# amathislab/BUCTD

Hardware: AMD Instinct MI355X
Metric: images/sec (train) BUCTD-CoAM-W48 384x288 (higher is better)
Workload: dtype f32 (3x3 convs: operands split exactly into 3 bf16 pieces, 6 bf16 MFMAs per product, fp32 accumulate - fp32-class); 1 GPU; BUCTD-CoAM-W48 (pose_hrnet_coam, ATT_MODULES [F,T,F,F], colored condition) 384x288 CrowdPose-14kpt full train step: fwd + JointsMSE + bwd + grad all-reduce + Adam + arg-max accuracy decode; global_batch=32, batch_per_gpu=32, input=N x 6 x 384 x 288 fp32, params=115581770, parallelism=dp1, hip_streams=4, conv_math=bf16x6, step_graph=False

## Files before the change

### buctd_amd/_C.py

```python
import ctypes as C
import os

import torch

_HERE = os.path.dirname(os.path.abspath(__file__))
LIB_PATH = os.path.join(_HERE, "lib", "libbuctd_hip.so")


class ConvDesc(C.Structure):
    _fields_ = [(n, C.c_int) for n in ("N", "H", "W", "Ci", "Co", "R", "S", "stride", "pad", "Ho", "Wo")]


class BasicBlockDesc(C.Structure):
    _fields_ = ([(n, C.c_int) for n in ("N", "H", "W", "C")] +
                [(n, C.c_void_p) for n in ("x", "w1_fwd", "w2_fwd", "w1_bwd", "w2_bwd", "gamma1", "beta1", "gamma2", "beta2",
                                           "running_mean1", "running_var1", "running_mean2", "running_var2")] +
                [(n, C.c_float) for n in ("eps1", "momentum1", "eps2", "momentum2")] +
                [(n, C.c_void_p) for n in ("z1", "z2", "y", "acc", "stat")])


class BasicBlockGrads(C.Structure):
    _fields_ = ([(n, C.c_void_p) for n in ("dy", "dz2", "dres", "dy1", "dz1", "dx", "dw1", "dw2", "dgamma1", "dbeta1",
                                           "dgamma2", "dbeta2")] +
                [(n, C.c_int) for n in ("acc_w1", "acc_w2", "acc_bn1", "acc_bn2")] +
                [("bn_acc", C.c_void_p), ("wg_ws", C.c_void_p), ("wg_ws_bytes", C.c_size_t)])


class BnAccIn(C.Structure):
    _fields_ = [("acc", C.c_void_p), ("rows", C.c_long), ("eps", C.c_float), ("momentum", C.c_float),
                ("mean_out", C.c_void_p), ("invstd_out", C.c_void_p), ("running_mean", C.c_void_p),
                ("running_var", C.c_void_p)]


class C3Conv(C.Structure):
    _fields_ = ([(n, C.c_int) for n in ("N", "H", "W", "Ci", "Co")] +
                [(n, C.c_void_p) for n in ("x", "wprep", "residual")] + [("relu", C.c_int)] +
                [(n, C.c_void_p) for n in ("y", "stats_acc")] + [("in_bn", C.POINTER(BnAccIn))] +
                [(n, C.c_void_p) for n in ("in_gamma", "in_beta")] + [("in_relu", C.c_int)] +
                [(n, C.c_void_p) for n in ("bn_z", "bn_y", "bn_mean", "bn_invstd", "bn_gamma", "bn_beta", "bn_acc")])


class C3ConvEval(C.Structure):
    _fields_ = ([(n, C.c_int) for n in ("N", "H", "W", "Ci", "Co")] +
                [(n, C.c_void_p) for n in ("x", "wprep", "scale", "shift", "residual")] + [("relu", C.c_int), ("y", C.c_void_p)])


class BnApplyItem(C.Structure):
    _fields_ = [("z", C.c_void_p), ("st", BnAccIn), ("gamma", C.c_void_p), ("beta", C.c_void_p), ("residual", C.c_void_p),
                ("relu", C.c_int), ("y", C.c_void_p), ("rows", C.c_long), ("C", C.c_int)]


class BnBwdItem(C.Structure):
    _fields_ = ([(n, C.c_void_p) for n in ("dy", "y", "z", "mean", "invstd", "gamma", "beta")] +
                [("relu", C.c_int), ("rows", C.c_long), ("C", C.c_int)] +
                [(n, C.c_void_p) for n in ("dz", "dres", "dgamma", "dbeta")] +
                [("accumulate", C.c_int), ("acc", C.c_void_p), ("acc_ready", C.c_int)])


class Wg3Conv(C.Structure):
    _fields_ = ([(n, C.c_int) for n in ("N", "H", "W", "Ci", "Co")] +
                [(n, C.c_void_p) for n in ("x", "dy", "dw")] + [("accumulate", C.c_int)] +
                [(n, C.c_void_p) for n in ("x_mean", "x_invstd", "x_gamma", "x_beta")] + [("x_relu", C.c_int)] +
                [("workspace", C.c_void_p), ("workspace_bytes", C.c_size_t)])


class MhaArgs(C.Structure):
    _fields_ = ([(n, C.c_int) for n in ("B", "T", "h", "dh")] +
                [(n, C.c_void_p) for n in ("q", "k", "v")] + [(n, C.c_int) for n in ("ldq", "ldk", "ldv")] +
                [("out", C.c_void_p), ("ldo", C.c_int), ("lse", C.c_void_p), ("scale", C.c_float), ("p_drop", C.c_float),
                 ("dout", C.c_void_p), ("lddo", C.c_int)] +
                [(n, C.c_void_p) for n in ("dq", "dk", "dv")] + [(n, C.c_int) for n in ("lddq", "lddk", "lddv")])


class AttnRowsArgs(C.Structure):
    _fields_ = ([(n, C.c_int) for n in ("B", "T", "h", "dh", "R")] + [("q", C.c_void_p), ("k", C.c_void_p)] +
                [("ldq", C.c_int), ("ldk", C.c_int), ("rows", C.c_void_p), ("scale", C.c_float), ("out", C.c_void_p),
                 ("out_heads", C.c_void_p)])


class RefineArgs(C.Structure):
    _fields_ = ([(n, C.c_void_p) for n in ("coords", "maxvals", "offset", "center", "scale", "box_score", "items",
                                           "cond_trunc", "cond_joints", "status", "hist_preds", "hist_score",
                                           "hist_box_score", "hist_keypoint_score", "hist_center", "hist_scale")] +
                [(n, C.c_int) for n in ("B", "K", "pass_", "passes", "heatmap_w", "heatmap_h", "crop_w", "crop_h")] +
                [(n, C.c_double) for n in ("margin", "aspect_ratio", "in_vis_thre", "scale_thre")])


class SampleGeomArgs(C.Structure):
    _fields_ = ([(n, C.c_void_p) for n in ("joints", "joints_vis", "cond", "cond_vis", "center", "scale", "bbox",
                                           "half_body", "draws", "bbox_draws", "flags", "pair", "items", "out_joints",
                                           "out_joints_vis", "out_cond", "out_cond_vis", "cond_trunc", "target_xy",
                                           "target_vis", "out_center", "out_scale", "out_rotation", "status")] +
                [(n, C.c_int) for n in ("B", "K", "crop_w", "crop_h", "keep_rect", "bbox_aug")] +
                [(n, C.c_double) for n in ("margin", "aspect_ratio", "scale_thre", "stride_x", "stride_y")])


class KptMatchArgs(C.Structure):
    _fields_ = ([(n, C.c_int) for n in ("images", "K", "n_thr", "n_area")] + [(n, C.c_long) for n in ("dt_total", "gt_total")] +
                [(n, C.c_void_p) for n in ("dt_offsets", "gt_offsets", "oks_offsets", "dt_kpts", "gt_kpts", "gt_area",
                                           "gt_bbox", "gt_flags", "sigmas", "thresholds", "area_ranges", "oks",
                                           "dt_matched", "dt_ignored")])


class VisCanvas(C.Structure):
    _fields_ = [("base", C.c_void_p), ("row_stride", C.c_long), ("H", C.c_int), ("W", C.c_int)]


class VisPoseArgs(C.Structure):
    _fields_ = ([(n, C.c_void_p) for n in ("canvases", "person_offsets", "persons", "joints", "skeleton", "palette",
                                           "tiles")] +
                [(n, C.c_int) for n in ("C", "P", "K", "L", "n_palette", "n_tiles", "canvas_h_max", "canvas_w_max",
                                        "style", "thickness", "radius")] +
                [("score_thresh", C.c_float), ("alpha256", C.c_int)])


VIS_POSE_PLAIN, VIS_POSE_PRETTY = 0, 1
# ... 62 lines not shown
    "buctd_bn_finalize": (_I, [_P, _P, _I, _I, _L, _I, _F, _F, _P, _P, _P, _P, _P]),
    "buctd_conv3x3_bf16x3_supported": (_I, [_I, _I, _I, _I, _I]),
    "buctd_conv3x3_bf16x3_stats_groups": (_I, [_I, _I, _I, _I, _I, _PI, _PI]),
    "buctd_conv3x3_bf16x3_prep_bytes": (_SZ, [_I, _I, _I]),
    "buctd_conv3x3_bf16x3_prep": (_I, [_I, _I, _P, _I, _P, _P]),
    "buctd_conv3x3_bf16x3_prep_batched": (_I, [_P, _I, _L, _P]),
    "buctd_conv3x3_bf16x3": (_I, [_I, _I, _I, _I, _I, _P, _P, _P, _P, _P, _P, _I, _P, _P, _P, _P]),
    "buctd_conv3x3_wgrad_bf16x3_supported": (_I, [_I, _I, _I, _I, _I]),
    "buctd_conv3x3_wgrad_bf16x3_workspace": (_SZ, [_I, _I, _I, _I, _I]),
    "buctd_conv3x3_wgrad_bf16x3": (_I, [_I, _I, _I, _I, _I, _P, _P, _P, _I, _P, _SZ, _P]),
    "buctd_conv3x3_bf16x6_supported": (_I, [_I, _I, _I, _I, _I]),
    "buctd_conv3x3_bf16x6_stats_groups": (_I, [_I, _I, _I, _I, _I, _PI, _PI]),
    "buctd_conv3x3_bf16x6_prep_bytes": (_SZ, [_I, _I, _I]),
    "buctd_conv3x3_bf16x6_prep": (_I, [_I, _I, _P, _I, _P, _P]),
    "buctd_conv3x3_bf16x6": (_I, [_I, _I, _I, _I, _I, _P, _P, _P, _P, _P, _P, _I, _P, _P, _P, _P]),
    "buctd_bn_bwd_from_partials": (_I, [_P, _P, _P, _P, _P, _P, _P, _I, _L, _I, _P, _I, _P, _P, _P, _P, _I, _P, _SZ, _P]),
    "buctd_conv3x3_wgrad_bf16x6_bnin": (_I, [_I, _I, _I, _I, _I, _P, _P, _P, _I, _P, _P, _P, _P, _I, _P, _SZ, _P]),
    "buctd_conv3x3_wgrad_bf16x6_supported": (_I, [_I, _I, _I, _I, _I]),
    "buctd_conv3x3_wgrad_bf16x6_workspace": (_SZ, [_I, _I, _I, _I, _I]),
    "buctd_conv3x3_wgrad_bf16x6": (_I, [_I, _I, _I, _I, _I, _P, _P, _P, _I, _P, _SZ, _P]),
    "buctd_bn_stats": (_I, [_P, _L, _I, _P, _PI, _PI, _P]),
    "buctd_bn_stats_groups": (_I, [_L, _I, _PI, _PI]),
    "buctd_bn_apply": (_I, [_P, _P, _P, _P, _P, _P, _I, _P, _L, _I, _P]),
    "buctd_bn_bwd_workspace": (_SZ, [_L, _I]),
    "buctd_bn_bwd": (_I, [_P, _P, _P, _P, _P, _P, _P, _I, _L, _I, _P, _P, _P, _P, _I, _P, _SZ, _P]),
    "buctd_bn_fold": (_I, [_P, _P, _P, _P, _F, _I, _P, _P, _P]),
    "buctd_bn_acc_bytes": (_SZ, [_I]),
    "buctd_bn_apply_acc": (_I, [_P, C.POINTER(BnAccIn), _P, _P, _P, _I, _P, _L, _I, _P]),
    "buctd_bn_bwd_acc": (_I, [_P, _P, _P, _P, _P, _P, _P, _I, _L, _I, _P, _P, _P, _P, _I, _P, _I, _P]),
    "buctd_conv3x3_bf16x6_acc": (_I, [_I] * 5 + [_P, _P, _P, _I, _P, _P, C.POINTER(BnAccIn), _P, _P, _I, _P]),
    "buctd_conv3x3_bf16x6_bnstat_acc": (_I, [_I] * 5 + [_P] * 12),
    "buctd_gconv_x6_fwd_acc": (_I, [_I] * 6 + [_P] * 6),
    "buctd_conv3x3_bf16x6_group": (_I, [_I, C.POINTER(C3Conv), _P]),
    "buctd_conv3x3_bf16x6_group_eval": (_I, [_I, C.POINTER(C3ConvEval), _P]),
    "buctd_conv3x3_bf16x6_group_workgroups": (_I, [_I, C.POINTER(C3Conv)]),
    "buctd_conv3x3_bf16x6_group_plan": (_I, [_I, C.POINTER(C3Conv), C.POINTER(C.c_int)]),
    "buctd_conv3x3_bf16x6_plan": (_I, [_I, _I, _I, _I, _I, _I, C.POINTER(C.c_int)]),
    "buctd_conv3x3_wgrad_bf16x6_plan": (_I, [_I, _I, _I, _I, _I, C.POINTER(C.c_int)]),
    "buctd_gconv_wgrad_x6_supported": (_I, [_I] * 6),
    "buctd_gconv_wgrad_x6_plan": (_I, [_I] * 6 + [C.POINTER(C.c_int)]),
    "buctd_gconv_wgrad_x6_workspace": (_SZ, [_I] * 6),
    "buctd_gconv_wgrad_x6": (_I, [_I] * 6 + [_P, _P, _P, _I, _P, _SZ, _P]),
    "buctd_bn_apply_acc_group": (_I, [_I, C.POINTER(BnApplyItem), _P]),
    "buctd_bn_bwd_acc_group": (_I, [_I, C.POINTER(BnBwdItem), _P]),
    "buctd_conv3x3_wgrad_bf16x6_group_workspace": (_SZ, [_I] * 6),
    "buctd_conv3x3_wgrad_bf16x6_group": (_I, [_I, C.POINTER(Wg3Conv), _P]),
    "buctd_conv3x3_wgrad_bf16x6_group_workgroups": (_I, [_I, C.POINTER(Wg3Conv)]),
    "buctd_conv3x3_wgrad_bf16x6_group_plan": (_I, [_I, C.POINTER(Wg3Conv), C.POINTER(C.c_int)]),
    "buctd_stream_fork": (_I, [_P, _P]),
    "buctd_basic_branches_fwd_train": (_I, [_I, _I, C.POINTER(BasicBlockDesc), _P]),
    "buctd_basic_branches_bwd": (_I, [_I, _I, C.POINTER(BasicBlockDesc), C.POINTER(BasicBlockGrads), _P, _P]),
    "buctd_basic_chain_fwd_train": (_I, [_I, C.POINTER(BasicBlockDesc), _P]),
    "buctd_basic_chain_bwd": (_I, [_I, C.POINTER(BasicBlockDesc), C.POINTER(BasicBlockGrads), _P, _P]),
    "buctd_x6_image_dims": (_I, [_I, _I, _I, _P, _P]),
    "buctd_x6_image_bytes": (C.c_size_t, [_I, _I, _I]),
    "buctd_x6_image": (_I, [_P, _I, _I, _I, _L, _L, _I, _L, _L, _I, _P, _P]),
    "buctd_x6_gemm": (_I, [_I, _I, _I, _P, _P, _P, _I, _F, _P, _L, _I, _L, _P]),
    "buctd_x6_gemm_plan": (_I, [_I, _I, _I, _PI]),
    "buctd_x6_gemm_tile": (_I, [_I, _I, _I, _I, _PI, _PI]),
    "buctd_x6_image_path": (_I, [_P, _I, _I, _I, _L, _L, _I, _L, _L, _I, _I, _I, _PI]),
    "buctd_add": (_I, [_P, _P, _P, _L, _I, _P]),
    "buctd_add_n": (_I, [C.POINTER(_P), _I, _P, _L, _P]),
    "buctd_mul": (_I, [_P, _P, _P, _L, _P]),
    "buctd_scale": (_I, [_P, _P, _F, _P, _L, _P]),
    "buctd_copy_channels": (_I, [_P, _L, _I, _I, _P, _I, _I, _I, _P]),
    "buctd_add_bcast": (_I, [_P, _P, _P, _L, _L, _P]),
    "buctd_batch_sum": (_I, [_P, _L, _L, _P, _I, _P]),
    "buctd_relu_bwd": (_I, [_P, _P, _P, _L, _P]),
    "buctd_colsum_workspace": (_SZ, [_L, _I]),
    "buctd_colsum": (_I, [_P, _L, _I, _P, _I, _P, _SZ, _P]),
    "buctd_nchw_to_nhwc": (_I, [_P, _I, _I, _I, _I, _I, _I, _P, _P]),
    "buctd_nhwc_to_nchw": (_I, [_P, _I, _I, _I, _I, _P, _P]),
    "buctd_fuse_sum": (_I, [C.POINTER(_P), _PI, _I, _I, _I, _I, _I, _I, _P, _P]),
    "buctd_fuse_sum_bwd": (_I, [_P, _P, _I, _I, _I, _I, _I, _P, _P]),
    "buctd_resize_bilinear": (_I, [_P, _I, _I, _I, _I, _I, _I, _I, _I, _P, _P]),
    "buctd_maxpool3x3s2_fwd": (_I, [_P, _I, _I, _I, _I, _P, _P, _P]),
    "buctd_maxpool3x3s2_bwd": (_I, [_P, _P, _I, _I, _I, _I, _P, _P]),
    "buctd_softmax_dropout_fwd": (_I, [_P, _L, _I, _F, _F, _U64, _P, _P, _P]),
    "buctd_softmax_dropout_bwd": (_I, [_P, _P, _L, _I, _F, _F, _U64, _P, _P]),
    "buctd_softmax_dropout_fwd_dseed": (_I, [_P, _L, _I, _F, _F, _P, _P, _P, _P]),
    "buctd_softmax_dropout_bwd_dseed": (_I, [_P, _P, _L, _I, _F, _F, _P, _P, _P]),
    "buctd_dropout": (_I, [_P, _P, _L, _F, _U64, _P]),
    "buctd_dropout_dseed": (_I, [_P, _P, _L, _F, _P, _P]),
    "buctd_dropout_seed_fill": (_I, [_P, _I, _U64, _U64, _P]),
    "buctd_attn_smallqk_supported": (_I, [_I, _I, _I]),
    "buctd_attn_smallqk_plan": (_I, [_I, _I, _I, _I, _F, _I, _PI]),
    "buctd_attn_smallqk_fwd": (_I, [_I, _I, _I, _I, _P, _P, _P, _F, _F, _U64, _I, _P, _P, _P, _P]),
    "buctd_attn_smallqk_bwd": (_I, [_I, _I, _I, _I, _P, _P, _P, _P, _P, _P, _P, _F, _F, _U64, _I, _P, _P, _P, _P, _P]),
    "buctd_attn_smallqk_fwd_dseed": (_I, [_I, _I, _I, _I, _P, _P, _P, _F, _F, _P, _I, _P, _P, _P, _P]),
    "buctd_attn_smallqk_bwd_dseed": (_I, [_I, _I, _I, _I, _P, _P, _P, _P, _P, _P, _P, _F, _F, _P, _I, _P, _P, _P, _P, _P]),
    "buctd_layernorm_fwd": (_I, [_P, _P, _P, _L, _I, _F, _P, _P, _P, _P]),
    "buctd_add_layernorm_fwd": (_I, [_P, _P, _P, _P, _L, _I, _F, _P, _P, _P, _P, _P]),
    "buctd_layernorm_bwd_workspace": (_SZ, [_L, _I]),
    "buctd_layernorm_bwd": (_I, [_P, _P, _P, _P, _P, _L, _I, _P, _P, _P, _I, _P, _SZ, _P]),
    "buctd_joints_mse": (_I, [_P, _P, _P, _I, _I, _I, _P, _P, _F, _P, _SZ, _P]),
    "buctd_joints_ohkm_mse_workspace": (_SZ, [_I, _I]),
    "buctd_joints_ohkm_mse": (_I, [_P, _P, _P, _I, _I, _I, _I, _P, _P, _F, _P, _SZ, _P]),
    "buctd_argmax_decode": (_I, [_P, _I, _I, _I, _P, _P, _P, _P]),
    "buctd_warp_affine_norm": (_I, [_P, _I, _I, _I, _P, _P, _P, _L, _P, _P]),
    "buctd_cond_render_into": (_I, [_P, _I, _P, _I, _I, _I, _I, _I, _I, _P, _L, _P, _SZ, _P]),
    "buctd_cond_geometry": (_I, [_P, _P, _P, _P, _I, _I, _P, _P, _P, _P]),
    "buctd_cond_mirror": (_I, [_P, _I, _P, _P, _I, _I, _I, _P, _P]),
    "buctd_mirror_rows": (_I, [_P, _L, _P, _L, _P, _I, _I, _I, _I, _I, _P]),
    "buctd_refine_step": (_I, [C.POINTER(RefineArgs), _P]),
    "buctd_sample_geometry": (_I, [C.POINTER(SampleGeomArgs), _P]),
    "buctd_synthesize_pose": (_I, [_P, _P, _P, _P, _P, _P, _I, _I, _I, C.c_ulonglong, _P, _P]),
# ... 117 lines not shown
```

### buctd_amd/models/hrnet_common.py

```python
import logging
import os

import torch

from .. import nn
from .. import ops

BN_MOMENTUM = 0.1
logger = logging.getLogger(__name__)


def conv3x3(in_planes, out_planes, stride=1):
    return nn.Conv2d(in_planes, out_planes, kernel_size=3, stride=stride, padding=1, bias=False)


class BasicBlock(nn.Module):
    expansion = 1

    def __init__(self, inplanes, planes, stride=1, downsample=None):
        super().__init__()
        self.conv1 = conv3x3(inplanes, planes, stride)
        self.bn1 = nn.BatchNorm2d(planes, momentum=BN_MOMENTUM)
        self.relu = nn.ReLU(inplace=True)
        self.conv2 = conv3x3(planes, planes)
# ... 128 lines not shown
            rows.append(nn.ModuleList(row))
        return nn.ModuleList(rows)

    def get_num_inchannels(self):
        return self.num_inchannels

    def _branches_grouped(self, x):
        nb = self.num_branches
        if not (self.training and torch.is_grad_enabled() and all(type(br) is BlockChain and len(br) > 1 for br in self.branches)):
            return None
        chains = []
        for br in self.branches:
            if not all(_native_block(m) and m.bn1.track_running_stats == br[0].bn1.track_running_stats for m in br):
                return None
            chains.append([_block_params(m) for m in br])
        xs = [x[i] for i in range(nb)]
        if not ops.group_branches_ok(xs, chains):
            return None
        parts = ops.group_branch_partition(nb)
        if len(parts) == 1:
            return list(ops.BasicBranchesFn.apply(chains[0][0][0], chains, *xs))
        outs = ops.fork_join([lambda p=p: ops.BasicBranchesFn.apply(chains[p[0]][0][0], [chains[i] for i in p], *[xs[i] for i in p])
                              for p in parts], [[xs[i] for i in p] for p in parts])
        ys = [None] * nb
        for p, o in zip(parts, outs):
            for i, y in zip(p, o):
                ys[i] = y
        return ys

    def _branches_grouped_eval(self, x):
        if self.training or torch.is_grad_enabled() or not all(type(br) is BlockChain and len(br) > 0 for br in self.branches):
            return None
        chains = []
        for br in self.branches:
            if not all(type(m) is BasicBlock and m.downsample is None and m.stride == 1 and m.conv1.bias is None
                       and m.conv2.bias is None and not m.bn1.training and not m.bn2.training
                       and m.bn1.running_mean is not None and m.bn2.running_mean is not None for m in br):
                return None
            chains.append([_block_params(m) for m in br])
        xs = [x[i] for i in range(self.num_branches)]
        if not ops.eval_branches_ok(xs, chains):
            return None
        return ops.basic_branches_eval(xs, chains)

    def forward(self, x):
        if self.num_branches == 1:
            return [self.branches[0](x[0])]
        xs = self._branches_grouped(x)
        if xs is None:
            xs = self._branches_grouped_eval(x)
        if xs is None:
            xs = ops.fork_join([lambda i=i: self.branches[i](x[i]) for i in range(self.num_branches)],
                               [x[i] for i in range(self.num_branches)])
        rows = list(enumerate(self.fuse_layers))
        fan = len(rows) > 1 and torch.is_grad_enabled() and any(t.requires_grad for t in xs)
        xr = [ops.FanOut.apply(xs[j], len(rows)) if fan and xs[j].is_cuda else [xs[j]] * len(rows)
              for j in range(self.num_branches)]

        def fuse_row(i, row):
            terms, shifts = [], []
            for j in range(self.num_branches):
                if j == i:
                    terms.append(xr[j][i])
                    shifts.append(0)
                elif j > i:
                    terms.append(row[j](xr[j][i]))
                    shifts.append(j - i)
                else:
                    terms.append(row[j](xr[j][i]))
                    shifts.append(0)
            return ops.FuseSum.apply(tuple(shifts), True, *terms)

        return ops.fork_join([lambda i=i, row=row: fuse_row(i, row) for i, row in rows], [xs for _ in rows], tag=1)


def make_transition_layer(pre, cur):
    layers = []
    for i in range(len(cur)):
        if i < len(pre):
            if cur[i] != pre[i]:
                layers.append(nn.ConvBN(nn.Conv2d(pre[i], cur[i], 3, 1, 1, bias=False), nn.BatchNorm2d(cur[i]),
                                        nn.ReLU(inplace=True)))
            else:
                layers.append(None)
        else:
            steps = []
            for j in range(i + 1 - len(pre)):
                cin = pre[-1]
                cout = cur[i] if j == i - len(pre) else cin
                steps.append(nn.ConvBN(nn.Conv2d(cin, cout, 3, 2, 1, bias=False), nn.BatchNorm2d(cout),
                                       nn.ReLU(inplace=True)))
            layers.append(nn.Chain(*steps))
    return nn.ModuleList(layers)


def make_stage(layer_config, num_inchannels, multi_scale_output=True):
    block = blocks_dict[layer_config["BLOCK"]]
    modules = []
    for i in range(layer_config["NUM_MODULES"]):
        mso = multi_scale_output or i != layer_config["NUM_MODULES"] - 1
        modules.append(HighResolutionModule(layer_config["NUM_BRANCHES"], block, layer_config["NUM_BLOCKS"],
                                            num_inchannels, layer_config["NUM_CHANNELS"],
                                            layer_config["FUSE_METHOD"], mso))
        num_inchannels = modules[-1].get_num_inchannels()
    return nn.Chain(*modules), num_inchannels


class HRNetTrunk(nn.Module):

    def build_trunk(self, extra, last_stage=4):
        self.conv1 = nn.Conv2d(3, 64, kernel_size=3, stride=2, padding=1, bias=False)
        self.bn1 = nn.BatchNorm2d(64, momentum=BN_MOMENTUM)
# ... 71 lines not shown
```

### buctd_amd/ops.py

```python
import ctypes as C
import math
import weakref

import torch

from . import _C
from ._C import ConvDesc, MatmulDesc, check, lib, ptr, stream_ptr

_capture = {"on": False, "events": set(), "allow_seeds": False, "seed_table": None, "seed_draws": 0}
_SEED_TABLE_SLOTS = 1024


def capturing():
    return _capture["on"]


def _new_event(stream=None):
    ev = torch.cuda.Event()
    ev.record(stream) if stream is not None else ev.record()
    if _capture["on"]:
        _capture["events"].add(id(ev))
        _capture.setdefault("keep", []).append(ev)
    return ev

# ... 1939 lines not shown
        return (None, None) + tuple(tmps[b][0, _Chain.DX] if ctx.needs_input_grad[2 + b] else None for b in range(nb))


class Conv(torch.autograd.Function):

    @staticmethod
    def forward(ctx, x, w, b, stride, pad, relu):
        y = conv_fwd(x, w, b, stride, pad, relu=relu)
        ctx.meta = (w, b, stride, pad, relu, tuple(x.shape))
        ctx.save_for_backward(x, y if relu else None)
        return y

    @staticmethod
    def backward(ctx, dy):
        w, b, stride, pad, relu, x_shape = ctx.meta
        x, y = ctx.saved_tensors
        dy = _contig(dy)
        if relu:
            dy = relu_bwd(dy, y)
        dx = conv_dgrad(dy, w, x_shape, stride, pad) if ctx.needs_input_grad[0] else None
        if w.requires_grad:
            dw, acc = grad_target(w)
            conv_wgrad_async(x, dy, w, stride, pad, dw, acc)
        if b is not None and b.requires_grad:
            db, acc = grad_target(b)
            colsum(dy, dy.shape[-1], db, acc)
        grad_done(w, b)
        return dx, None, None, None, None, None


class FuseSum(torch.autograd.Function):

    @staticmethod
    def forward(ctx, shifts, relu, *terms):
        out = fuse_sum(list(terms), list(shifts), relu)
        ctx.shifts, ctx.relu = shifts, relu
        ctx.save_for_backward(out if relu else None)
        return out

    @staticmethod
    def backward(ctx, dy):
        (y,) = ctx.saved_tensors
        dy = _contig(dy)
        cache = {}
        grads = []
        for j, s in enumerate(ctx.shifts):
            if not ctx.needs_input_grad[2 + j]:
                grads.append(None)
                continue
            if s not in cache:
                cache[s] = fuse_sum_bwd(dy, y, s) if s > 0 or ctx.relu else dy
            grads.append(cache[s])
        return (None, None, *grads)


class AddN(torch.autograd.Function):

    @staticmethod
    def forward(ctx, a, b, c):
        out = add(a, b)
        if c is not None:
            out = add(out, c, out=out)
        ctx.n = 3 if c is not None else 2
        return out

    @staticmethod
    def backward(ctx, dy):
        return dy, dy, (dy if ctx.n == 3 else None)


def add_n(terms):
    acc = terms[0]
    k = 1
    while k < len(terms):
        group = [acc] + list(terms[k:k + 3])
        k += 3
        out = torch.empty_like(acc)
        arr = (C.c_void_p * len(group))(*[t.data_ptr() for t in group])
        check(lib().buctd_add_n(arr, len(group), ptr(out), acc.numel(), stream_ptr()), "add_n")
        acc = out
    return acc


class FanOut(torch.autograd.Function):

    @staticmethod
    def forward(ctx, x, n):
        return tuple(x.view_as(x) for _ in range(n))

    @staticmethod
    def backward(ctx, *grads):
        gs = [_contig(g) for g in grads if g is not None]
        if not gs:
            return None, None
        return (gs[0] if len(gs) == 1 else add_n(gs)), None


class ToNCHW(torch.autograd.Function):
    @staticmethod
    def forward(ctx, x):
        return nhwc_to_nchw(x)

    @staticmethod
    def backward(ctx, dy):
        return nchw_to_nhwc(_contig(dy))

# ... 397 lines not shown
```

### include/buctd_hip.h

```cpp
#ifndef BUCTD_HIP_H
#define BUCTD_HIP_H
#include <stddef.h>
#include <stdint.h>

#ifdef __cplusplus
extern "C" {
#endif

int buctd_version(void);
const char* buctd_last_error(void);

typedef struct {
  int N, H, W, Ci;
  int Co, R, S;
  int stride, pad;
  int Ho, Wo;
} buctd_conv_desc;

int buctd_conv2d_fwd_thin(const buctd_conv_desc* d);
int buctd_conv2d_fwd(const buctd_conv_desc* d, const float* x, const float* w, const float* bias,
                     const float* scale, const float* shift, const float* residual, int relu, float* y,
                     float* stats_partials, void* stream);
int buctd_conv2d_dgrad(const buctd_conv_desc* d, const float* dy, const float* w, const float* bias, float* dx,
                       float* stats_partials, void* stream);
// ... 248 lines not shown
int buctd_flipback_avg(const float* a, const float* b, const int32_t* perm, int N, int K, int H, int W, int shift,
                       float* out, void* stream);

int buctd_gconv_x6_supported(int kind, int N, int H, int W, int Ci, int Co, int dir);
size_t buctd_gconv_x6_prep_bytes(int kind, int Ci, int Co, int dir);
int buctd_gconv_x6_prep(int kind, int Ci, int Co, const float* w, int dir, void* wprep, void* stream);
size_t buctd_gconv_x6_prep_item_bytes(void);
int buctd_gconv_x6_prep_item(int kind, int Ci, int Co, const float* w, int dir, void* wprep, void* item_host);
int buctd_gconv_x6_prep_batched(const void* items_device, int n, void* stream);
int buctd_gconv_x6_stats_groups(int kind, int N, int H, int W, int Ci, int Co, int* ngroups, int* rows_per_group);
int buctd_gconv_x6_fwd(int kind, int N, int H, int W, int Ci, int Co, const float* x, const void* wprep, const float* bias,
                       const float* scale, const float* shift, const float* residual, int relu, float* y,
                       float* stats_partials, int* stats_counts, void* stream);
int buctd_gconv_x6_fwd_acc(int kind, int N, int H, int W, int Ci, int Co, const float* x, const void* wprep, const float* bias,
                           float* y, void* stats_acc, void* stream);
int buctd_gconv_x6_dgrad(int kind, int N, int H, int W, int Ci, int Co, const float* dy, const void* wprep,
                         const float* residual, float* dx, void* stream);
int buctd_gconv_x6_plan(int kind, int dir, int N, int H, int W, int Ci, int Co, int flags, int* out);
int buctd_gconv_wgrad_x6_supported(int kind, int N, int H, int W, int Ci, int Co);
int buctd_gconv_wgrad_x6_plan(int kind, int N, int H, int W, int Ci, int Co, int* out);
size_t buctd_gconv_wgrad_x6_workspace(int kind, int N, int H, int W, int Ci, int Co);
int buctd_gconv_wgrad_x6(int kind, int N, int H, int W, int Ci, int Co, const float* x, const float* dy, float* dw,
                         int accumulate, void* workspace, size_t workspace_bytes, void* stream);

typedef struct {
  int N, H, W, C;
  const float* x;
  const void *w1_fwd, *w2_fwd;
  const void *w1_bwd, *w2_bwd;
  const float *gamma1, *beta1, *gamma2, *beta2;
  float *running_mean1, *running_var1, *running_mean2, *running_var2;
  float eps1, momentum1, eps2, momentum2;
  float *z1, *z2, *y;
  void* acc;
  float* stat;
} buctd_basic_block;
typedef struct {
  const float* dy;
  float *dz2, *dres, *dy1, *dz1;
  float* dx;
  float *dw1, *dw2, *dgamma1, *dbeta1, *dgamma2, *dbeta2;
  int acc_w1, acc_w2, acc_bn1, acc_bn2;
  void* bn_acc;
  void* wg_ws; size_t wg_ws_bytes;
} buctd_basic_block_grads;
int buctd_basic_chain_fwd_train(int n, const buctd_basic_block* blocks, void* stream);
int buctd_basic_chain_bwd(int n, const buctd_basic_block* blocks, const buctd_basic_block_grads* grads, void* stream,
                          void* side_stream);

int buctd_basic_branches_fwd_train(int nb, int n, const buctd_basic_block* blocks, void* stream);
int buctd_basic_branches_bwd(int nb, int n, const buctd_basic_block* blocks, const buctd_basic_block_grads* grads, void* stream,
                             void* side_stream);

int buctd_stream_fork(void* from, void* to);

int buctd_x6_image_dims(int V, int K, int role, int* Vpad, int* Kpad);
size_t buctd_x6_image_bytes(int V, int K, int role);
int buctd_x6_image(const float* src, int V, int K, int vg, long vgs, long vs, int kg, long kgs, long ks, int role,
                   void* image, void* stream);
int buctd_x6_gemm(int M, int N, int K, const void* a_image, const void* b_image, const float* bias, int bias_axis,
                  float alpha, float* C, long ldc, int Nc, long gsc, void* stream);
int buctd_x6_gemm_plan(int M, int N, int K, int* out);
int buctd_x6_gemm_tile(int lin, int gx, int gy, int row_major, int* bx, int* by);
int buctd_x6_image_path(const float* src, int V, int K, int vg, long vgs, long vs, int kg, long kgs, long ks, int role,
                        int v, int k0, int* vector);

int buctd_adam_step(float* p, const float* g, float* m, float* v, long n, float lr, float beta1, float beta2,
                    float eps, int step, float gscale, void* stream);
int buctd_sgd_step(float* p, const float* g, float* momentum_buf, long n, float lr, float momentum, float weight_decay,
                   int nesterov, int first_step, float gscale, void* stream);
int buctd_adam_step_dscale(float* p, const float* g, float* m, float* v, long n, float lr, float beta1, float beta2,
                           float eps, int step, float gscale, const float* coef, void* stream);
int buctd_sgd_step_dscale(float* p, const float* g, float* momentum_buf, long n, float lr, float momentum,
                          float weight_decay, int nesterov, int first_step, float gscale, const float* coef, void* stream);

#define BUCTD_STEP_MAX_GROUPS 16
#define BUCTD_STEP_CHUNK 16384
typedef struct {
  long start;
  int len;
  int group;
} buctd_step_chunk;
typedef struct {
  float lr, beta1, beta2, eps, weight_decay;
  int decoupled;
  int step;
} buctd_adam_group;
typedef struct {
  float lr, momentum, weight_decay;
  int nesterov;
} buctd_sgd_group;
long buctd_step_chunks(const long* runs, const int* run_group, int nruns, buctd_step_chunk* out);
int buctd_adam_step_groups(float* p, const float* g, float* m, float* v, const buctd_step_chunk* chunks_device, long nchunks,
                           const buctd_adam_group* groups, int ngroups, float gscale, const float* coef, void* stream);
int buctd_sgd_step_groups(float* p, const float* g, float* buf, const buctd_step_chunk* chunks_device, long nchunks,
                          const buctd_sgd_group* groups, int ngroups, float gscale, const float* coef, void* stream);

#define BUCTD_GRAD_SUMSQ_CHUNK 8192
size_t buctd_grad_sumsq_workspace(const long* runs, int nruns);
int buctd_grad_sumsq(const float* g, const long* runs, int nruns, double* sumsq, void* workspace, size_t workspace_bytes,
                     void* stream);
int buctd_grad_clip_coef(const double* sumsq, double gscale, double max_norm, float* coef, float* total_norm, void* stream);
int buctd_grad_segment_stats(const float* g, const long* spans, int P, double* abs_mean, double* norm, void* stream);

int buctd_ema_update(const float* p, float* avg, long n, float w, void* stream);
typedef struct {
// ... 242 lines not shown
```

Baseline: 513.9 images/s.

## Run each HRNet fuse row as one native fwd/bwd call with grouped BN

Adds a native fuse-row path that runs every conv+BN chain feeding one HRNet fuse-layer output, plus the final sum, in a single C call per direction. Forward advances all terms step by step so their BN applies can share one grouped launch. Backward groups the BN backward kernels the same way and sends weight gradients to a side stream while data gradients stay on the main stream. The aim is to cut Python/autograd dispatch and kernel launch count in the fuse layers, at the cost of a large new code path with its own validity checks and fallback conditions.

```diff
diff --git a/buctd_amd/_C.py b/buctd_amd/_C.py
--- a/buctd_amd/_C.py
+++ b/buctd_amd/_C.py
@@ -62,6 +62,28 @@
                 [(n, C.c_void_p) for n in ("x", "dy", "dw")] + [("accumulate", C.c_int)] +
                 [(n, C.c_void_p) for n in ("x_mean", "x_invstd", "x_gamma", "x_beta")] + [("x_relu", C.c_int)] +
                 [("workspace", C.c_void_p), ("workspace_bytes", C.c_size_t)])
+
+
+class FuseStep(C.Structure):
+    _fields_ = ([("d", ConvDesc)] + [(n, C.c_void_p) for n in ("x", "w", "wp_fwd", "wp_bwd")] + [("wg_kind", C.c_int)] +
+                [(n, C.c_void_p) for n in ("gamma", "beta", "running_mean", "running_var")] +
+                [("eps", C.c_float), ("momentum", C.c_float), ("relu", C.c_int)] +
+                [(n, C.c_void_p) for n in ("z", "y", "acc", "part")] + [("ngroups", C.c_int), ("rows_per_group", C.c_int)] +
+                [(n, C.c_void_p) for n in ("mean", "invstd")])
+
+
+class FuseStepGrads(C.Structure):
+    _fields_ = ([(n, C.c_void_p) for n in ("dy", "dz", "dx", "dw", "dgamma", "dbeta")] + [("acc_w", C.c_int), ("acc_bn", C.c_int)] +
+                [("bn_acc", C.c_void_p), ("wg_ws", C.c_void_p), ("wg_ws_bytes", C.c_size_t)])
+
+
+class FuseTerm(C.Structure):
+    _fields_ = [("shift", C.c_int), ("nsteps", C.c_int), ("first", C.c_int), ("t", C.c_void_p)]
+
+
+class FuseRow(C.Structure):
+    _fields_ = ([(n, C.c_int) for n in ("N", "H", "W", "C", "relu", "nterms")] + [("terms", FuseTerm * 4)] +
+                [("y", C.c_void_p), ("dy", C.c_void_p), ("g", C.c_void_p * 4)])
 
 
 class MhaArgs(C.Structure):
@@ -230,6 +252,8 @@
     "buctd_basic_branches_bwd": (_I, [_I, _I, C.POINTER(BasicBlockDesc), C.POINTER(BasicBlockGrads), _P, _P]),
     "buctd_basic_chain_fwd_train": (_I, [_I, C.POINTER(BasicBlockDesc), _P]),
     "buctd_basic_chain_bwd": (_I, [_I, C.POINTER(BasicBlockDesc), C.POINTER(BasicBlockGrads), _P, _P]),
+    "buctd_fuse_row_fwd_train": (_I, [C.POINTER(FuseRow), C.POINTER(FuseStep), _P]),
+    "buctd_fuse_row_bwd": (_I, [C.POINTER(FuseRow), C.POINTER(FuseStep), C.POINTER(FuseStepGrads), _P, _P]),
     "buctd_x6_image_dims": (_I, [_I, _I, _I, _P, _P]),
     "buctd_x6_image_bytes": (C.c_size_t, [_I, _I, _I]),
     "buctd_x6_image": (_I, [_P, _I, _I, _I, _L, _L, _I, _L, _L, _I, _P, _P]),
diff --git a/buctd_amd/csrc/fuse_row.hip b/buctd_amd/csrc/fuse_row.hip
--- /dev/null
+++ b/buctd_amd/csrc/fuse_row.hip
@@ -0,0 +1,163 @@
+#include "common.h"
+#include "../../include/buctd_hip.h"
+
+#define FR_TRY(call)        \
+  do {                      \
+    const int rc_ = (call); \
+    if (rc_) return rc_;    \
+  } while (0)
+
+#define FR_MAX_STEPS 16
+
+static int gc_kind_of(const buctd_conv_desc& d) {
+  if (d.R == 1 && d.S == 1 && d.stride == 1 && d.pad == 0) return 1;
+  if (d.R == 3 && d.S == 3 && d.stride == 2 && d.pad == 1) return 2;
+  return 0;
+}
+
+static long out_rows(const buctd_conv_desc& d) { return (long)d.N * d.Ho * d.Wo; }
+
+static int row_check(bool fwd, const buctd_fuse_row* row, const buctd_fuse_step* steps, const char* who, int* maxlen) {
+  BUCTD_CHECK_ARG(row && row->nterms >= 2 && row->nterms <= BUCTD_FUSE_MAX_TERMS && row->y && row->N > 0 && row->H > 0 &&
+                      row->W > 0 && row->C > 0,
+                  "%s: bad row (2..%d terms)", who, BUCTD_FUSE_MAX_TERMS);
+  int len = 0, total = 0;
+  for (int j = 0; j < row->nterms; ++j) {
+    const buctd_fuse_term& t = row->terms[j];
+    BUCTD_CHECK_ARG((t.t || !fwd) && t.nsteps >= 0 && t.shift >= 0 && t.shift < 31 && (t.nsteps == 0 || (steps && t.first >= 0)),
+                    "%s: bad term %d", who, j);
+    BUCTD_CHECK_ARG((row->H >> t.shift) << t.shift == row->H && (row->W >> t.shift) << t.shift == row->W,
+                    "%s: term %d: %d x %d is no multiple of 2^%d", who, j, row->H, row->W, t.shift);
+    total += t.nsteps;
+    BUCTD_CHECK_ARG(total <= FR_MAX_STEPS, "%s: more than %d steps", who, FR_MAX_STEPS);
+    for (int k = 0; k < t.nsteps; ++k) {
+      const buctd_fuse_step& S = steps[t.first + k];
+      BUCTD_CHECK_ARG(gc_kind_of(S.d) && S.x && S.w && S.gamma && S.beta && S.z && (S.y || !fwd) && S.mean && S.invstd &&
+                          S.d.Co % 4 == 0 && S.d.Co <= 1024,
+                      "%s: term %d step %d: a 1x1 or stride-2 3x3 convolution with all its tensors, Co %% 4 == 0, Co <= 1024", who,
+                      j, k);
+      BUCTD_CHECK_ARG(!fwd || (S.wp_fwd ? S.acc != nullptr : (S.part && S.ngroups > 0 && S.rows_per_group > 0)),
+                      "%s: term %d step %d: a gathered forward needs its accumulator, a generic one its partials", who, j, k);
+      BUCTD_CHECK_ARG(k == 0 || ((steps[t.first + k - 1].y == S.x || !fwd) && steps[t.first + k - 1].d.Co == S.d.Ci &&
+                                 steps[t.first + k - 1].d.Ho == S.d.H && steps[t.first + k - 1].d.Wo == S.d.W),
+                      "%s: term %d step %d does not read the step in front of it", who, j, k);
+    }
+    if (t.nsteps) {
+      const buctd_fuse_step& L = steps[t.first + t.nsteps - 1];
+      BUCTD_CHECK_ARG((L.y == t.t || !fwd) && L.d.N == row->N && L.d.Ho == row->H >> t.shift && L.d.Wo == row->W >> t.shift &&
+                          L.d.Co == row->C,
+                      "%s: term %d: the chain does not end in the term the row sums", who, j);
+    }
+    if (t.nsteps > len) len = t.nsteps;
+  }
+  *maxlen = len;
+  return BUCTD_OK;
+}
+
+extern "C" int buctd_fuse_row_fwd_train(const buctd_fuse_row* row, const buctd_fuse_step* steps, void* stream) {
+  int maxlen;
+  FR_TRY(row_check(true, row, steps, "buctd_fuse_row_fwd_train", &maxlen));
+  for (int k = 0; k < maxlen; ++k) {
+    for (int j = 0; j < row->nterms; ++j) {
+      if (row->terms[j].nsteps <= k) continue;
+      const buctd_fuse_step& S = steps[row->terms[j].first + k];
+      const buctd_conv_desc& d = S.d;
+      if (S.wp_fwd)
+        FR_TRY(buctd_gconv_x6_fwd_acc(gc_kind_of(d), d.N, d.H, d.W, d.Ci, d.Co, S.x, S.wp_fwd, nullptr, S.z, S.acc, stream));
+      else
+        FR_TRY(buctd_conv2d_fwd(&d, S.x, S.w, nullptr, nullptr, nullptr, nullptr, 0, S.z, S.part, stream));
+    }
+    buctd_bn_apply_item ap[BUCTD_FUSE_MAX_TERMS];
+    int n = 0;
+    for (int j = 0; j < row->nterms; ++j) {
+      if (row->terms[j].nsteps <= k) continue;
+      const buctd_fuse_step& S = steps[row->terms[j].first + k];
+      const long rows = out_rows(S.d);
+      if (!S.wp_fwd) {
+        FR_TRY(buctd_bn_finalize(S.part, nullptr, S.ngroups, S.rows_per_group, rows, S.d.Co, S.eps, S.momentum, S.mean, S.invstd,
+                                 S.running_mean, S.running_var, stream));
+        FR_TRY(buctd_bn_apply(S.z, S.mean, S.invstd, S.gamma, S.beta, nullptr, S.relu, S.y, rows, S.d.Co, stream));
+        continue;
+      }
+      buctd_bn_apply_item& a = ap[n++];
+      a.z = S.z;
+      a.st = buctd_bn_acc_in{S.acc, rows, S.eps, S.momentum, S.mean, S.invstd, S.running_mean, S.running_var};
+      a.gamma = S.gamma; a.beta = S.beta; a.residual = nullptr; a.relu = S.relu; a.y = S.y;
+      a.rows = rows; a.C = S.d.Co;
+    }
+    if (n == 1)
+      FR_TRY(buctd_bn_apply_acc(ap->z, &ap->st, ap->gamma, ap->beta, nullptr, ap->relu, ap->y, ap->rows, ap->C, stream));
+    else if (n)
+      FR_TRY(buctd_bn_apply_acc_group(n, ap, stream));
+  }
+  const float* terms[BUCTD_FUSE_MAX_TERMS];
+  int shifts[BUCTD_FUSE_MAX_TERMS];
+  for (int j = 0; j < row->nterms; ++j) {
+    terms[j] = row->terms[j].t;
+    shifts[j] = row->terms[j].shift;
+  }
+  return buctd_fuse_sum(terms, shifts, row->nterms, row->N, row->H, row->W, row->C, row->relu, row->y, stream);
+}
+
+extern "C" int buctd_fuse_row_bwd(const buctd_fuse_row* row, const buctd_fuse_step* steps, const buctd_fuse_step_grads* grads,
+                                  void* stream, void* side_stream) {
+  int maxlen;
+  FR_TRY(row_check(false, row, steps, "buctd_fuse_row_bwd", &maxlen));
+  BUCTD_CHECK_ARG(row->dy && (grads || !maxlen), "buctd_fuse_row_bwd: null pointer");
+  for (int j = 0; j < row->nterms; ++j) {
+    const buctd_fuse_term& t = row->terms[j];
+    for (int k = 0; k < t.nsteps; ++k) {
+      const buctd_fuse_step_grads& G = grads[t.first + k];
+      BUCTD_CHECK_ARG(G.dy && G.dz && G.dw && G.dgamma && G.dbeta && G.bn_acc && (G.wg_ws || !G.wg_ws_bytes),
+                      "buctd_fuse_row_bwd: null pointer in term %d step %d", j, k);
+      BUCTD_CHECK_ARG(k == 0 || grads[t.first + k - 1].dy == G.dx, "buctd_fuse_row_bwd: term %d step %d: dx is not the upstream "
+                      "gradient of the step in front", j, k);
+    }
+    if (t.nsteps)
+      BUCTD_CHECK_ARG(t.shift < BUCTD_FUSE_MAX_TERMS && row->g[t.shift] && grads[t.first + t.nsteps - 1].dy == row->g[t.shift],
+                      "buctd_fuse_row_bwd: term %d does not read the gradient of its shift", j);
+  }
+  void* side = side_stream ? side_stream : stream;
+  for (int s = 0; s < BUCTD_FUSE_MAX_TERMS; ++s)
+    if (row->g[s])
+      FR_TRY(buctd_fuse_sum_bwd(row->dy, row->relu ? row->y : nullptr, s, row->N, row->H, row->W, row->C, row->g[s], stream));
+  for (int r = 0; r < maxlen; ++r) {
+    int at[BUCTD_FUSE_MAX_TERMS], n = 0;
+    buctd_bn_bwd_item bi[BUCTD_FUSE_MAX_TERMS];
+    for (int j = 0; j < row->nterms; ++j) {
+      const buctd_fuse_term& t = row->terms[j];
+      if (t.nsteps <= r) continue;
+      const int i = at[n] = t.first + t.nsteps - 1 - r;
+      const buctd_fuse_step& S = steps[i];
+      const buctd_fuse_step_grads& G = grads[i];
+      bi[n++] = buctd_bn_bwd_item{G.dy, nullptr, S.z, S.mean, S.invstd, S.gamma, S.relu ? S.beta : nullptr, S.relu, out_rows(S.d),
+                                  S.d.Co, G.dz, nullptr, G.dgamma, G.dbeta, G.acc_bn, G.bn_acc, 0};
+    }
+    if (n == 1)
+      FR_TRY(buctd_bn_bwd_acc(bi->dy, bi->y, bi->z, bi->mean, bi->invstd, bi->gamma, bi->beta, bi->relu, bi->rows, bi->C, bi->dz,
+                              bi->dres, bi->dgamma, bi->dbeta, bi->accumulate, bi->acc, 0, stream));
+    else
+      FR_TRY(buctd_bn_bwd_acc_group(n, bi, stream));
+    FR_TRY(buctd_stream_fork(stream, side));
+    for (int m = 0; m < n; ++m) {
+      const buctd_fuse_step& S = steps[at[m]];
+      const buctd_fuse_step_grads& G = grads[at[m]];
+      const buctd_conv_desc& d = S.d;
+      if (S.wg_kind)
+        FR_TRY(buctd_gconv_wgrad_x6(S.wg_kind, d.N, d.H, d.W, d.Ci, d.Co, S.x, G.dz, G.dw, G.acc_w, G.wg_ws, G.wg_ws_bytes, side));
+      else
+        FR_TRY(buctd_conv2d_wgrad(&d, S.x, G.dz, G.dw, G.acc_w, G.wg_ws, G.wg_ws_bytes, side));
+    }
+    for (int m = 0; m < n; ++m) {
+      const buctd_fuse_step& S = steps[at[m]];
+      const buctd_fuse_step_grads& G = grads[at[m]];
+      const buctd_conv_desc& d = S.d;
+      if (!G.dx) continue;
+      if (S.wp_bwd)
+        FR_TRY(buctd_gconv_x6_dgrad(gc_kind_of(d), d.N, d.H, d.W, d.Ci, d.Co, G.dz, S.wp_bwd, nullptr, G.dx, stream));
+      else
+        FR_TRY(buctd_conv2d_dgrad(&d, G.dz, S.w, nullptr, G.dx, nullptr, stream));
+    }
+  }
+  return BUCTD_OK;
+}
diff --git a/buctd_amd/models/hrnet_common.py b/buctd_amd/models/hrnet_common.py
--- a/buctd_amd/models/hrnet_common.py
+++ b/buctd_amd/models/hrnet_common.py
@@ -204,12 +204,38 @@
         if xs is None:
             xs = ops.fork_join([lambda i=i: self.branches[i](x[i]) for i in range(self.num_branches)],
                                [x[i] for i in range(self.num_branches)])
+        return self.fuse(xs)
+
+    def _row_terms(self, i, row):
+        terms = []
+        for j in range(self.num_branches):
+            if j == i:
+                terms.append(None)
+                continue
+            steps = [row[j]] if j > i else list(row[j])
+            if not all(type(m) is nn.ConvBN and type(m[0]) is nn.Conv2d and m[0].bias is None and m[0].groups == 1
+                       and m[0].dilation == (1, 1) and m[0].kernel_size[:1] + m[0]._geom() in ((1, 1, 0), (3, 2, 1))
+                       and m[1].training for m in steps):
+                return None
+            for m in steps:
+                nn._as_channels_last_(m[0].weight)
+            terms.append([(m[0].weight, m[1], m._relu) for m in steps])
+        return terms
+
+    def fuse(self, xs):
         rows = list(enumerate(self.fuse_layers))
         fan = len(rows) > 1 and torch.is_grad_enabled() and any(t.requires_grad for t in xs)
         xr = [ops.FanOut.apply(xs[j], len(rows)) if fan and xs[j].is_cuda else [xs[j]] * len(rows)
               for j in range(self.num_branches)]
 
+        native = self.training and torch.is_grad_enabled()
+
         def fuse_row(i, row):
+            plain = self._row_terms(i, row) if native else None
+            if plain is not None:
+                xi = [xr[j][i] for j in range(self.num_branches)]
+                if ops.fuse_row_ok(i, plain, xi):
+                    return ops.FuseRowFn.apply(plain[1 if i == 0 else 0][0][0], i, plain, *xi)
             terms, shifts = [], []
             for j in range(self.num_branches):
                 if j == i:
diff --git a/buctd_amd/ops.py b/buctd_amd/ops.py
--- a/buctd_amd/ops.py
+++ b/buctd_amd/ops.py
@@ -2015,6 +2015,202 @@
                 cache[s] = fuse_sum_bwd(dy, y, s) if s > 0 or ctx.relu else dy
             grads.append(cache[s])
         return (None, None, *grads)
+
+
+def _fuse_step_plan(d):
+    def plan():
+        kind = _gconv_kind(d)
+        if not kind or not bn_acc_ok(d.Co) or lib().buctd_conv2d_fwd_thin(C.byref(d)) == 1:
+            return None
+        fwd_g, bwd_g = _gconv_ok(d, 0), _gconv_ok(d, 1)
+        wg_kind, need = kind, -1
+        if lib().buctd_gconv_wgrad_x6_supported(kind, d.N, d.H, d.W, d.Ci, d.Co) == 1:
+            need = int(lib().buctd_gconv_wgrad_x6_workspace(kind, d.N, d.H, d.W, d.Ci, d.Co))
+        if need < 0:
+            wg_kind, need = 0, int(lib().buctd_conv2d_wgrad_workspace(C.byref(d)))
+        ng, rpg = C.c_int(), C.c_int()
+        if not fwd_g:
+            check(lib().buctd_conv2d_stats_groups(C.byref(d), 0, C.byref(ng), C.byref(rpg)), "stats_groups")
+        return fwd_g, bwd_g, wg_kind, need, ng.value, rpg.value
+    return _memo(("fuserow",) + _dkey(d), plan)
+
+
+def _fuse_row_descs(i, terms, xs):
+    N, H, W, Cn = xs[i].shape
+    out = []
+    for j, (t, x) in enumerate(zip(terms, xs)):
+        if j == i:
+            out.append(None)
+            continue
+        s = max(j - i, 0)
+        if (H >> s) << s != H or (W >> s) << s != W or len(t) > 3:
+            return None
+        shape, ds = tuple(x.shape), []
+        for (w, bn, relu) in t:
+            ws = _wshape(w)
+            if ws[1] != shape[3]:
+                return None
+            k = ws[2]
+            d = conv_desc(shape, ws, 1 if k == 1 else 2, 0 if k == 1 else 1)
+            if _fuse_step_plan(d) is None:
+                return None
+            ds.append(d)
+            shape = (d.N, d.Ho, d.Wo, d.Co)
+        if shape != (N, H >> s, W >> s, Cn):
+            return None
+        out.append(ds)
+    return out
+
+
+def fuse_row_ok(i, terms, xs):
+    if not (2 <= len(xs) <= 4 and native_chain_ok(tuple(xs[i].shape))):
+        return False
+    if not all(x.is_cuda and x.dim() == 4 and x.dtype == torch.float32 and x.is_contiguous() for x in xs):
+        return False
+    for j, t in enumerate(terms):
+        if j == i:
+            continue
+        for (w, bn, relu) in t:
+            if not (w.dim() == 4 and w.shape[2] == w.shape[3] and w.shape[2] in (1, 3) and w.requires_grad and bn.weight.requires_grad
+                    and bn.bias.requires_grad and w.is_contiguous(memory_format=torch.channels_last)):
+                return False
+    return _fuse_row_descs(i, terms, xs) is not None
+
+
+class FuseRowFn(torch.autograd.Function):
+
+    @staticmethod
+    def _fill(row, steps, i, terms, descs, xs, zs, ys, stats):
+        N, H, W, Cn = xs[i].shape
+        row.N, row.H, row.W, row.C, row.relu, row.nterms = N, H, W, Cn, 1, len(xs)
+        at = 0
+        plans = []
+        for j, x in enumerate(xs):
+            T = row.terms[j]
+            T.shift = max(j - i, 0)
+            if j == i:
+                T.nsteps, T.first, T.t = 0, 0, x.data_ptr()
+                continue
+            T.nsteps, T.first = len(terms[j]), at
+            xin = x.data_ptr()
+            for (w, bn, relu), d in zip(terms[j], descs[j]):
+                S = steps[at]
+                plan = _fuse_step_plan(d)
+                plans.append(plan)
+                kind = _gconv_kind(d)
+                S.d, S.x, S.w = d, xin, weight_rsc(w).data_ptr()
+                S.wp_fwd = _gconv_prepared(w, kind, 0).data_ptr() if plan[0] else None
+                S.wp_bwd = _gconv_prepared(w, kind, 1).data_ptr() if plan[1] else None
+                S.wg_kind = plan[2]
+                S.gamma, S.beta = bn.weight.data_ptr(), bn.bias.data_ptr()
+                S.eps, S.momentum, S.relu = bn.eps, 0.1 if bn.momentum is None else bn.momentum, int(bool(relu))
+                S.z = zs[at].data_ptr()
+                S.y = xin = ys[at].data_ptr() if ys[at] is not None else None
+                S.mean, S.invstd = stats[at][0].data_ptr(), stats[at][1].data_ptr()
+                at += 1
+            T.t = xin
+        return plans
+
+    @staticmethod
+    def forward(ctx, w_first, i, terms, *xs):
+        dev = xs[i].device
+        descs = _fuse_row_descs(i, terms, xs)
+        flat = [(t, d) for j in range(len(xs)) if j != i for t, d in zip(terms[j], descs[j])]
+        n = len(flat)
+        zs = [torch.empty((d.N, d.Ho, d.Wo, d.Co), dtype=torch.float32, device=dev) for _, d in flat]
+        ys = [torch.empty_like(z) for z in zs]
+        stats = [torch.empty((2, d.Co), dtype=torch.float32, device=dev) for _, d in flat]
+        row, steps = _C.FuseRow(), (_C.FuseStep * n)()
+        plans = FuseRowFn._fill(row, steps, i, terms, descs, xs, zs, ys, stats)
+        keep = []
+        for S, plan, ((w, bn, relu), d) in zip(steps, plans, flat):
+            if plan[0]:
+                S.acc = AccRef(d.Co, dev).ptr
+            else:
+                part = torch.empty((plan[4], d.Co, 2), dtype=torch.float32, device=dev)
+                keep.append(part)
+                S.part, S.ngroups, S.rows_per_group = part.data_ptr(), plan[4], plan[5]
+            if bn.track_running_stats:
+                S.running_mean, S.running_var = bn.running_mean.data_ptr(), bn.running_var.data_ptr()
+                _count_batch(bn)
+        y = torch.empty_like(xs[i])
+        row.y = y.data_ptr()
+        check(lib().buctd_fuse_row_fwd_train(C.byref(row), steps, stream_ptr()), "fuse_row_fwd_train")
+        ctx.meta = (i, terms, len(xs))
+        inner, at = [], 0
+        for j in range(len(xs)):
+            if j != i:
+                inner += ys[at:at + len(terms[j]) - 1]
+                at += len(terms[j])
+        ctx.save_for_backward(y, *xs, *zs, *stats, *inner)
+        return y
+
+    @staticmethod
+    def backward(ctx, dy):
+        i, terms, nb = ctx.meta
+        saved = ctx.saved_tensors
+        y, xs = saved[0], saved[1:1 + nb]
+        n = sum(len(terms[j]) for j in range(nb) if j != i)
+        zs, stats, inner = saved[1 + nb:1 + nb + n], saved[1 + nb + n:1 + nb + 2 * n], list(saved[1 + nb + 2 * n:])
+        ys = []
+        for j in range(nb):
+            if j != i:
+                ys += [inner.pop(0) for _ in range(len(terms[j]) - 1)] + [None]
+        dev = y.device
+        need = ctx.needs_input_grad[3:]
+        dy = _contig(dy)
+        descs = _fuse_row_descs(i, terms, xs)
+        row, steps, grads = _C.FuseRow(), (_C.FuseStep * n)(), (_C.FuseStepGrads * n)()
+        plans = FuseRowFn._fill(row, steps, i, terms, descs, xs, zs, ys, stats)
+        N, H, W, Cn = y.shape
+        g = [None] * 4
+        for j in range(nb):
+            s = max(j - i, 0)
+            if g[s] is None and (j != i or need[j]):
+                g[s] = torch.empty((N, H >> s, W >> s, Cn), dtype=torch.float32, device=dev)
+                row.g[s] = g[s].data_ptr()
+        row.y, row.dy = y.data_ptr(), dy.data_ptr()
+        main = torch.cuda.current_stream(dev)
+        use_side = _side["on"]
+        side = _side_stream(dev) if use_side else main
+        wg_ws = workspace_on(side, max(p[3] for p in plans), dev)
+        dxs, used, done = [None] * nb, [dy], []
+        at = 0
+        for j in range(nb):
+            if j == i:
+                dxs[j] = g[0] if need[j] else None
+                continue
+            L = len(terms[j])
+            up = g[max(j - i, 0)]
+            for k in range(L - 1, -1, -1):
+                (w, bn, relu), G, d = terms[j][k], grads[at + k], descs[j][k]
+                dz = torch.empty_like(zs[at + k])
+                dx = torch.empty((d.N, d.H, d.W, d.Ci), dtype=torch.float32, device=dev) if (k > 0 or need[j]) else None
+                dw, acc_w = grad_target(w)
+                dg, acc_g = grad_target(bn.weight)
+                db, acc_b = grad_target(bn.bias)
+                assert acc_g == acc_b
+                weight_rsc(dw)
+                G.dy, G.dz, G.dx = up.data_ptr(), dz.data_ptr(), dx.data_ptr() if dx is not None else None
+                G.dw, G.dgamma, G.dbeta, G.acc_w, G.acc_bn = dw.data_ptr(), dg.data_ptr(), db.data_ptr(), int(acc_w), int(acc_g)
+                G.bn_acc = AccRef(d.Co, dev).ptr
+                G.wg_ws, G.wg_ws_bytes = wg_ws.data_ptr(), wg_ws.numel()
+                used += [dz, up]
+                done.append((L - 1 - k, bn.weight, bn.bias, w))
+                up = dx
+            dxs[j] = up if need[j] else None
+            at += L
+        check(lib().buctd_fuse_row_bwd(C.byref(row), steps, grads, main.cuda_stream, side.cuda_stream if use_side else None),
+              "fuse_row_bwd")
+        if use_side:
+            for t in list(xs) + [u for u in ys if u is not None] + used:
+                t.record_stream(side)
+            _queue_join()
+        elif _branch["on"]:
+            _queue_join()
+        for _, bw, bb, w in sorted(done, key=lambda e: e[0]):
+            grad_done(bw, bb, w)
+        return (None, None, None) + tuple(dxs)
 
 
 class AddN(torch.autograd.Function):
diff --git a/include/buctd_hip.h b/include/buctd_hip.h
--- a/include/buctd_hip.h
+++ b/include/buctd_hip.h
@@ -324,6 +324,51 @@
 int buctd_basic_branches_bwd(int nb, int n, const buctd_basic_block* blocks, const buctd_basic_block_grads* grads, void* stream,
                              void* side_stream);
 
+typedef struct {
+  buctd_conv_desc d;
+  const float* x;
+  const float* w;
+  const void *wp_fwd, *wp_bwd;
+  int wg_kind;
+  const float *gamma, *beta;
+  float *running_mean, *running_var;
+  float eps, momentum;
+  int relu;
+  float *z, *y;
+  void* acc;
+  float* part;
+  int ngroups, rows_per_group;
+  float *mean, *invstd;
+} buctd_fuse_step;
+typedef struct {
+  const float* dy;
+  float* dz;
+  float* dx;
+  float *dw, *dgamma, *dbeta;
+  int acc_w, acc_bn;
+  void* bn_acc;
+  void* wg_ws; size_t wg_ws_bytes;
+} buctd_fuse_step_grads;
+#define BUCTD_FUSE_MAX_TERMS 4
+typedef struct {
+  int shift;
+  int nsteps;
+  int first;
+  const float* t;
+} buctd_fuse_term;
+typedef struct {
+  int N, H, W, C;
+  int relu;
+  int nterms;
+  buctd_fuse_term terms[BUCTD_FUSE_MAX_TERMS];
+  float* y;
+  const float* dy;
+  float* g[BUCTD_FUSE_MAX_TERMS];
+} buctd_fuse_row;
+int buctd_fuse_row_fwd_train(const buctd_fuse_row* row, const buctd_fuse_step* steps, void* stream);
+int buctd_fuse_row_bwd(const buctd_fuse_row* row, const buctd_fuse_step* steps, const buctd_fuse_step_grads* grads, void* stream,
+                       void* side_stream);
+
 int buctd_stream_fork(void* from, void* to);
 
 int buctd_x6_image_dims(int V, int K, int role, int* Vpad, int* Kpad);
```

Result: no change. 513.7 images/s (-0.0%).
